# sdoira/U96-SLAM

Measured on AMD Instinct MI355X. Metric: Mpix-disparities/s, higher is better.
Workload: dtype u8

## Files before the change

### u96-slam_amd/csrc/sbm_api.hip

```cpp
#include <stdio.h>
#include <stdlib.h>
#include <string.h>

#include <algorithm>
#include <mutex>
#include <new>

#include "sbm_handle.h"

using namespace sbm;

enum BmStage { kBmPrefilter, kBmSad, kBmBorder, kBmLr, kBmSpeckle, kBmTotal, kBmStageCount };
enum BmMark { kBmBegin, kBmPrefiltered, kBmMatched, kBmChecked, kBmEnd, kBmMarkCount };
static const char* const kBmNames[] = {"prefilter", "sad", "border", "lrcheck", "speckle", "total"};
StageTable sbm::bm_stages() { return stage_table<kBmStageCount, 0>(kBmNames); }
static_assert(kBmMarkCount == sbm_handle::kMarks, "the ring holds one event per mark");

extern "C" {

void sbm_params_default(sbm_params* p, int num_disparities, int block_size) {
  if (!p) return;
  memset(p, 0, sizeof(*p));
  p->prefilter_type = SBM_PREFILTER_XSOBEL;
  p->prefilter_size = 9;
// ... 275 lines not shown
    pl->sad = wide ? kSadWide : kSadGeneric;
    snprintf(pl->kernel, sizeof(pl->kernel), "%s",
             !wide ? "sad_generic_kernel" : (pl->in_envelope ? "sad_wide_kernel [in-place accumulate unavailable]" : "sad_wide_kernel"));
  }
  pl->speckle = p.speckle_range >= 0 && p.speckle_window_size > 0;
  if (pl->speckle) {
    speckle_plan(g, p.speckle_window_size, p.speckle_range, &pl->spk);
    size_t part[4];
    SpeckleScratch::bytes(g.n, g.W, g.H, part);
    for (int i = 0; i < 4; i++) pl->spk_bytes[i] = (long long)part[i];
  }
}

extern "C" {

static int ensure_scratch(sbm_handle* h, int n, int W, int H, int pitch, bool need_cost, bool need_speckle) {
  auto& s = h->bm;
  const bool fits = n <= s.n && W == s.W && H == s.H && pitch == s.pitch && s.pf_l.p;
  if (!fits) {
    HIPCHK(h, hipStreamSynchronize(h->stream));
    release_set(s);
    const size_t npix = (size_t)n * W * H, pfbytes = (size_t)n * pitch * H + 4096;
    HIPCHK(h, s.pf_l.grow(pfbytes, h->stream));
    HIPCHK(h, s.pf_r.grow(pfbytes, h->stream));
    HIPCHK(h, s.disp_pre.grow(npix * sizeof(int16_t), h->stream));
    HIPCHK(h, hipMemsetAsync(s.pf_l.p, 0, pfbytes, h->stream));
    HIPCHK(h, hipMemsetAsync(s.pf_r.p, 0, pfbytes, h->stream));
    s.n = n; s.W = W; s.H = H; s.pitch = pitch;
  }
  const size_t npix = (size_t)s.n * W * H;
  if (need_cost) HIPCHK(h, s.cost.grow(npix * sizeof(int32_t), h->stream));
  HIPCHK(h, s.lr_keys.grow(lr_keys_bytes(s.n, W, H, need_cost), h->stream));
  if (need_speckle) HIPCHK(h, s.spk.ensure(s.n, W, H, h->stream));
  return SBM_OK;
}

static inline void mark(sbm_handle* h, BmMark i) {
  if (h->instr) hipEventRecord(h->ev[h->calls % sbm_handle::kRing][i], h->stream);
}

static void collect_profile(sbm_handle* h) {
  unsigned nrec = std::min<unsigned>(h->calls, sbm_handle::kRing), first = 0;
  if (h->profiling == 1 && h->calls > 0) { first = (h->calls - 1) % sbm_handle::kRing; nrec = 1; }
  static const BmStage kStage[kBmMarkCount - 1] = {kBmPrefilter, kBmSad, kBmLr, kBmSpeckle};
  float acc[kBmMarkCount - 1] = {}, tot = 0.f;
  for (unsigned r = first; r < first + nrec; r++) {
    for (int i = 0; i < kBmMarkCount - 1; i++) {
      float ms = 0.f;
// ... 9 lines not shown

int sbm_compute_device(sbm_handle* h, int n, const void* d_left, const void* d_right, int width, int height,
                       void* d_disp, int sync) {
  if (!h || !d_left || !d_right || !d_disp) return SBM_ERR_NULL;
  if (n <= 0) return SBM_ERR_BATCH;
  const sbm_params& p = h->p;
  BmPlan pl;
  const int st = bm_plan_geom(p, n, width, height, &pl);
  if (st != SBM_OK) return st;
  DeviceScope dscope(h->device);
  HIPCHK(h, dscope.enter());
  bool inplace = false;
  if (pl.in_envelope) HIPCHK(h, mqsad_inplace_ok(h->stream, &inplace));
  bm_plan_launches(p, inplace, &pl);
  const Geom& g = pl.g;
  const int st2 = ensure_scratch(h, n, width, height, g.pitch, g.want_cost, pl.speckle);
  if (st2 != SBM_OK) return st2;
  h->last = g; h->have_last = true;
  if (pl.any_rows) snprintf(h->last_kernel, sizeof(h->last_kernel), "%s", pl.kernel);

  const uint8_t* dl = (const uint8_t*)d_left;
  const uint8_t* dr = (const uint8_t*)d_right;
  uint8_t *pf_l = h->bm.pf_l.as<uint8_t>(), *pf_r = h->bm.pf_r.as<uint8_t>();
  int16_t* disp_pre = h->bm.disp_pre.as<int16_t>();
  int32_t* cost = h->bm.cost.as<int32_t>();
  int16_t* out = (int16_t*)d_disp;

  h->instr = h->profiling && h->ev_ok && (h->profiling != 3 || (h->ncall & 3u) == 0);
  mark(h, kBmBegin);
  if (pl.any_rows) {
    if (p.prefilter_type == SBM_PREFILTER_XSOBEL) {
      HIPCHK(h, launch_prefilter(dl, dr, pf_l, pf_r, g, h->stream));
    } else {
      HIPCHK(h, h->bm.vsum.grow((size_t)2 * h->bm.n * width * height * sizeof(uint16_t), h->stream));
      HIPCHK(h, launch_prefilter_norm(dl, dr, pf_l, pf_r, h->bm.vsum.as<uint16_t>(), g, p.prefilter_size, h->stream));
    }
  }
  mark(h, kBmPrefiltered);
  if (pl.sad == kSadFast) {
    HIPCHK(h, launch_sad_fast(pf_l, pf_r, disp_pre, cost, pl, h->stream));
    if (pl.wide_borders) {
      HIPCHK(h, launch_sad_wide(pf_l, pf_r, disp_pre, cost, g, pl.wide_l[0], pl.wide_l[1], h->stream));
      HIPCHK(h, launch_sad_wide(pf_l, pf_r, disp_pre, cost, g, pl.wide_r[0], pl.wide_r[1], h->stream));
    }
  } else if (pl.sad == kSadWide) {
    HIPCHK(h, launch_sad_wide(pf_l, pf_r, disp_pre, cost, g, 0, g.xend, h->stream));
  } else if (pl.sad == kSadGeneric) {
    HIPCHK(h, launch_sad_generic(pf_l, pf_r, disp_pre, cost, g, 0, g.xend, h->stream));
  }
  mark(h, kBmMatched);
  HIPCHK(h, launch_lrcheck(disp_pre, cost, out, h->bm.lr_keys.as<unsigned long long>(), g, p.disp12_max_diff, h->stream));
  mark(h, kBmChecked);
  if (pl.speckle) HIPCHK(h, launch_speckle(out, h->bm.spk, g, pl.spk, p.speckle_window_size, h->stream));
  mark(h, kBmEnd);
  if (h->instr) h->calls++;
// ... 153 lines not shown
    return SBM_OK;
  }
  if (which == 3) {
    if (dst_bytes < npix * sizeof(int16_t)) return SBM_ERR_SIZE;
    HIPCHK(h, hipMemcpy(dst, h->bm.disp_pre.p, npix * sizeof(int16_t), hipMemcpyDeviceToHost));
    int16_t* d = (int16_t*)dst;
    for (int i = 0; i < g.n; i++)
      for (int y = 0; y < g.H; y++) {
        int16_t* row = d + ((size_t)i * g.H + y) * g.W;
        const bool live = y >= g.row0 && y < g.row1;
        for (int x = 0; x < g.W; x++)
          if (!live || x < g.lofs || x >= g.lofs + g.xend) row[x] = (int16_t)g.filtered;
      }
    return SBM_OK;
  }
  return SBM_ERR_UNSUPPORTED;
}

}
```

### u96-slam_amd/csrc/sbm_common.h

```cpp
#pragma once
#include <hip/hip_runtime.h>
#include <stdint.h>

#include "../../include/sbm.h"

#include <stdlib.h>

namespace sbm {

inline int env_switch(const char* name, int dflt) {
  const char* e = getenv(name);
  return e ? atoi(e) : dflt;
}

struct Geom {
  int W, H;
  int n;
  int pitch;
  int padl;
  int plane;
  int nd, mindisp, wsz, w2, cap;
  int lofs, rofs, width1, xend;
  int tex, uniq;
  int filtered;
// ... 61 lines not shown
};
int bm_plan_geom(const sbm_params& p, int n, int W, int H, BmPlan* pl);
void bm_plan_launches(const sbm_params& p, bool inplace_ok, BmPlan* pl);
inline int bm_plan(const sbm_params& p, int n, int W, int H, bool inplace_ok, BmPlan* pl) {
  const int st = bm_plan_geom(p, n, W, H, pl);
  if (st == SBM_OK) bm_plan_launches(p, inplace_ok, pl);
  return st;
}

bool sad_fast_supported(const Geom& g);
hipError_t mqsad_inplace_ok(hipStream_t s, bool* ok);
constexpr int kFastNdMax = 512;
bool sad_fast_borders_in_launch(const Geom& g);
int sad_fast_pfshift(const Geom& g);
void sad_fast_plan(BmPlan* pl);
hipError_t launch_sad_fast(const uint8_t* pf_l, const uint8_t* pf_r, int16_t* disp, int32_t* cost, BmPlan& pl, hipStream_t s);

constexpr int kLrLdsCols = 8192;
inline size_t lr_keys_bytes(int n, int W, int H, bool do_lr) {
  return do_lr && W > kLrLdsCols ? (size_t)n * H * W * sizeof(unsigned long long) : 0;
}
hipError_t launch_lrcheck(const int16_t* disp_pre, const int32_t* cost, int16_t* disp_out, unsigned long long* keys,
                          const Geom& g, int disp12_max_diff, hipStream_t s);

constexpr int kSpkMaxSeg = 4, kSpkRecordPad = 288, kSpkSeamPad = 512;
void speckle_plan(const Geom& g, int max_size, int max_diff, SpkPlan* k);

hipError_t launch_prefilter_dense(const uint8_t* d_src, uint8_t* d_dst, int n, int W, int H, int rtl, int cap,
                                  hipStream_t s);
hipError_t launch_rect_map(const sbm_rect_cam& cam, int W, int H, int16_t* d_map, hipStream_t s);
hipError_t launch_rect_remap(const uint8_t* d_src, const int16_t* d_map, uint8_t* d_dst, int n, int W, int H,
// ... 23 lines not shown
```

### u96-slam_amd/csrc/sbm_handle.h

```cpp
#pragma once
#include <string.h>

#include "sbm_common.h"

#define HIPCHK(h, call)                         \
  do {                                          \
    hipError_t e_ = (call);                     \
    if (e_ != hipSuccess) {                     \
      (h)->last_hip = (int)e_;                  \
      return e_ == hipErrorOutOfMemory ? SBM_ERR_NOMEM : SBM_ERR_HIP; \
    }                                           \
  } while (0)

struct DeviceScope {
  int prev, dev;
  bool have;
  explicit DeviceScope(int d) : prev(-1), dev(d), have(false) { have = hipGetDevice(&prev) == hipSuccess; }
  hipError_t enter() { return (have && prev == dev) ? hipSuccess : hipSetDevice(dev); }
  ~DeviceScope() {
    if (have && prev != dev) hipSetDevice(prev);
  }
};

namespace sbm {
// ... 88 lines not shown

}

struct sbm_handle {
  sbm_params p;
  int device;
  hipStream_t stream;
  int last_hip;
  struct {
    int n, W, H, pitch;
    sbm::DevBuf pf_l, pf_r;
    sbm::DevBuf disp_pre;
    sbm::DevBuf cost;
    sbm::DevBuf lr_keys;
    sbm::DevBuf vsum;
    sbm::SpeckleScratch spk;
    sbm::StageClock clock;
    template <class F> void each(F f) { f(pf_l); f(pf_r); f(disp_pre); f(cost); f(lr_keys); f(vsum); spk.each(f); }
  } bm;
  struct {
    int n, W, H;
    int gen;
    sbm::DevBuf rec, flag, xs_l, xs_r;
    template <class F> void each(F f) { f(rec); f(flag); f(xs_l); f(xs_r); }
  } fp;
  struct {
    int n, W, H;
    sbm::DevBuf l, r, d;
    sbm::DevBuf zc_cnt;
    template <class F> void each(F f) { f(l); f(r); f(d); f(zc_cnt); }
  } st;
  uint8_t* pin;
  size_t pin_bytes;
// ... 106 lines not shown
```

### u96-slam_amd/csrc/sbm_sad_fast.hip

```cpp
#include <string.h>

#include "sbm_sad_fast_kernel.h"

namespace sbm {

__global__ void __launch_bounds__(256) mqsad_inplace_selftest_kernel(unsigned* bad) {
  unsigned long long st = (unsigned long long)(blockIdx.x * 256 + threadIdx.x) * 0x9E3779B97F4A7C15ull + 88172645463325252ull;
  auto rnd = [&]() { st ^= st << 13; st ^= st >> 7; st ^= st << 17; return st; };
  unsigned nbad = 0;
  for (int it = 0; it < 64; it++) {
    unsigned long long accA[4], accR[4], win[4];
    const unsigned pat = (unsigned)rnd() & ((it & 1) ? 0x00ffffffu : 0x000000ffu);
#pragma unroll
    for (int q = 0; q < 4; q++) { accA[q] = accR[q] = rnd() & 0x3fff3fff3fff3fffull; win[q] = rnd(); }
#pragma unroll
    for (int r = 0; r < 3; r++)
#pragma unroll
      for (int q = 0; q < 4; q++) {
        accR[q] = __builtin_amdgcn_mqsad_pk_u16_u8(win[(q + r) & 3], pat, accR[q]);
        asm volatile("v_mqsad_pk_u16_u8 %0, %1, %2, %0" : "+v"(accA[q]) : "v"(win[(q + r) & 3]), "v"(pat));
      }
#pragma unroll
    for (int q = 0; q < 4; q++) nbad += accA[q] != accR[q];
  }
// ... 59 lines not shown
  if (g.row0 < g.w2 || g.row1 > g.H - g.w2 || g.row1 <= g.row0) return false;
  if ((long)g.plane * 4 >= (1L << 31)) return false;
  const int xhi = std::min(g.W - g.lofs - 1, g.W - g.rofs - g.nd);
  if (xhi - g.w2 + 1 <= g.w2) return false;
  return true;
}

static hipError_t sad_fast_dispatch(BmPlan& pl, const FastArgs* a, hipStream_t s) {
  switch (pl.g.wsz) {
    case 15: return launch_nd<5, 3>(pl, a, s);
    case 21: return launch_nd<7, 3>(pl, a, s);
    default: return launch_sad_fast_pw1(pl, a, s);
  }
}

void sad_fast_plan(BmPlan* pl) {
  const Geom& g = pl->g;
  FastPlan& a = pl->f;
  const int xhi = std::min(g.W - g.lofs - 1, g.W - g.rofs - g.nd);
  a.xc0 = g.w2; a.xc1 = xhi - g.w2 + 1;
  const int pw = g.wsz % 3 == 0 ? 3 : 1;
  const int nv = 64 - (g.wsz - pw);
  const int cs3_env = env_switch("SBM_FAST_CS3", 1);
  const int ncols = a.xc1 - a.xc0;
  const int nv3 = 64 - (g.wsz / 3 - 1);
  int triples = 0;
  if (pw == 3 && cs3_env) {
    triples = ncols / (3 * nv3);
    if (ncols - triples * 3 * nv3 > 2 * nv) triples++;
  }
  a.strips3 = 3 * triples;
  const int rem = std::max(0, ncols - triples * 3 * nv3);
  const int strips = a.strips3 + (rem + nv - 1) / nv;
  const int rows = g.row1 - g.row0;
  const int round1 = g.nd <= 256 ? 1536 : (g.nd <= 384 ? 1024 : 768);
  constexpr double kSegC = 0.196;
  int nseg = 1;
  {
    const double prime = 0.2 * (g.wsz - 1);
    const double slots = g.nd <= 64 ? 4096.0 : (g.nd <= 128 ? 3072.0 : (double)round1);
    nseg = (int)(std::sqrt(kSegC * slots * rows / ((double)strips * g.n * prime)) + 0.5);
    nseg = std::max(1, std::min(nseg, std::max(1, rows / g.wsz)));
  }
  constexpr int kSmallRows = 8;
  constexpr long kFill = 5000;
  const int maxseg = std::max(nseg, std::min(64, rows / kSmallRows));
  const long per_seg = (long)strips * g.n;
  if (per_seg * maxseg * (g.nd > 128 ? (g.nd + 127) / 128 : 1) < 1800) {
    nseg = std::max(nseg, (int)std::min<long>(maxseg, 1023 / per_seg));
  } else {
    const int nseg1 = nseg;
    while (per_seg * nseg < kFill && nseg < maxseg) nseg++;
    if (g.nd > 128 && per_seg * nseg > round1 && 2 * per_seg * nseg < 3 * round1) nseg = std::max(nseg1, (int)((long)round1 * 1450 / 1536 / per_seg));
  }
  nseg = std::min(nseg, 64);
  int ns = 0;
  a.segrow[0] = g.row0;
  if (nseg < 3) {
    const int seg = (rows + nseg - 1) / nseg;
    for (int y = g.row0; y < g.row1; y += seg) a.segrow[++ns] = std::min(y + seg, g.row1);
  } else {
    const double unit = rows / (nseg - 1.5);
    double acc = 0;
    for (int k = 0; k < nseg; k++) {
      const double wgt = k < nseg - 3 ? 1.0 : (k == nseg - 3 ? 0.75 : (k == nseg - 2 ? 0.5 : 0.25));
      acc += wgt * unit;
      const int y = k == nseg - 1 ? g.row1 : std::min(g.row1, g.row0 + (int)(acc + 0.5));
      if (y > a.segrow[ns]) a.segrow[++ns] = y;
    }
  }
  nseg = ns;
  a.strips = strips; a.nseg = nseg;
  {
    const long maxs = (long)g.wsz * g.wsz * 2 * g.cap;
    a.uniq_plain = 8 * ((maxs * g.uniq / 100 + 1) << g.pfshift) <= 65535;
  }
  a.split = (long)strips * nseg * g.n < 1024;
  sad_fast_dispatch(*pl, nullptr, nullptr);
}

hipError_t launch_sad_fast(const uint8_t* pf_l, const uint8_t* pf_r, int16_t* disp, int32_t* cost, BmPlan& pl, hipStream_t s) {
  const Geom& g = pl.g;
  const FastPlan& f = pl.f;
  FastArgs a;
  a.pf_l = pf_l; a.pf_r = pf_r; a.disp = disp; a.cost = g.want_cost ? reinterpret_cast<uint16_t*>(cost) : nullptr;
  a.W = g.W; a.H = g.H; a.pitch = g.pitch; a.padl = g.padl; a.plane = g.plane;
  a.nd = g.nd; a.mindisp = g.mindisp; a.lofs = g.lofs; a.rofs = g.rofs; a.tex = g.tex << g.pfshift; a.uniq = g.uniq;
  a.filtered = g.filtered; a.capb = (g.cap << g.pfshift) + kPfBias; a.pfshift = g.pfshift;
  a.row0 = g.row0; a.row1 = g.row1;
  static_assert(sizeof(a.segrow) == sizeof(f.segrow), "");
  memcpy(a.segrow, f.segrow, sizeof(a.segrow));
  a.strips = f.strips; a.nseg = f.nseg; a.npairs = g.n; a.strips3 = f.strips3; a.uniq_plain = f.uniq_plain;
  a.xc0 = f.xc0; a.xc1 = f.xc1;
  a.bord = f.bord; a.bnw = f.bnw; a.bseg = f.bseg; a.nbseg = f.nbseg;
  return sad_fast_dispatch(pl, &a, s);
}

}
```

### u96-slam_amd/csrc/sbm_sad_fast_core.h

```cpp
#pragma once
#include <stdio.h>
#include <stdlib.h>

#include <algorithm>
#include <cmath>
#include <mutex>
#include <type_traits>

#include "sbm_common.h"

namespace sbm {

typedef unsigned int u32;
typedef unsigned long long u64;
typedef unsigned short u16x2 __attribute__((ext_vector_type(2)));
typedef unsigned int u32x4 __attribute__((ext_vector_type(4)));

struct FastArgs {
  const uint8_t* pf_l;
  const uint8_t* pf_r;
  int16_t* disp;
  uint16_t* cost;
  int W, H, pitch, padl, plane;
  int nd, mindisp, lofs, rofs, tex, uniq, filtered, capb;
  int row0, row1;
  int segrow[66];
  int strips, nseg, npairs;
  int strips3;
  int uniq_plain;
  int xc0, xc1;
  int pfshift;
  int bord;
  int bnw;
  int bseg, nbseg;
};

__device__ __forceinline__ u32 pk_sub_sat(u32 a, u32 b) {
  u16x2 r = __builtin_elementwise_sub_sat(__builtin_bit_cast(u16x2, a), __builtin_bit_cast(u16x2, b));
  return __builtin_bit_cast(u32, r);
}
__device__ __forceinline__ u32 pk_add_sat(u32 a, u32 b) {
  u16x2 r = __builtin_elementwise_add_sat(__builtin_bit_cast(u16x2, a), __builtin_bit_cast(u16x2, b));
  return __builtin_bit_cast(u32, r);
}
__device__ __forceinline__ u32 pk_min(u32 a, u32 b) {
  u16x2 r = __builtin_elementwise_min(__builtin_bit_cast(u16x2, a), __builtin_bit_cast(u16x2, b));
  return __builtin_bit_cast(u32, r);
}
__device__ __forceinline__ u32 umin3(u32 a, u32 b, u32 c) {
  u32 r;
  asm("v_min3_u32 %0, %1, %2, %3" : "=v"(r) : "v"(a), "v"(b), "v"(c));
  return r;
}

extern __shared__ __attribute__((aligned(16))) uint4 fast_lds[];

#include "sbm_sad_border_wave.h"

constexpr int kFastPrioExchange = 2;

template <int NDW, int NTERM, int PW, int CS>
struct FastLds {
  static constexpr int NQ = NDW / 4;
  static constexpr int NCH = (NQ + 15) / 16;
  static constexpr int NSLOT = ((CS * 63 + 4 + 16 * (4 * (NCH - 1) + 3) + 1) + 63) / 64 * 64;
  static constexpr int KS = CS == 3 ? 1 : PW;
  static constexpr int XS = 64 + KS * (NTERM - 1);
  static_assert(CS == 1 || (CS == 3 && PW == 3), "column stride 3 goes with 3-column sums");
// ... 162 lines not shown
```

### u96-slam_amd/csrc/sbm_sad_fast_kernel.h

```cpp
#pragma once
#include "sbm_sad_fast_core.h"
#include "sbm_sad_fast_strip.h"

namespace sbm {

template <int NDW, int NWAVES, int NTERM, int PW, bool EXACT_ND, bool DUAL>
__global__ void __launch_bounds__(64 * NWAVES) __attribute__((amdgpu_waves_per_eu(NDW > 64 ? 3 : (NWAVES > 2 ? 5 : 4))))
sad_fast_kernel(FastArgs a) {
  const int bpp = a.strips;
  int strip, segi, pair;
  {
    if constexpr (NDW * NWAVES <= 256) {
    if ((int)blockIdx.x < a.bord * a.nbseg) {
      using BL = BorderLds<(PW * NTERM) / 2, NDW * NWAVES>;
      const int bseg = blockIdx.x / a.bord, b = blockIdx.x - bseg * a.bord;
      const int wv = NWAVES > 1 ? __builtin_amdgcn_readfirstlane(threadIdx.x >> 6) : 0;
      const int wi = b * NWAVES + wv;
      if (wi < a.bnw) sad_border_wave<(PW * NTERM) / 2, NDW * NWAVES>(a, reinterpret_cast<unsigned char*>(fast_lds) + wv * BL::BYTES, bseg, wi);
      return;
    }
    }
    const int sid = blockIdx.x - a.bord * a.nbseg;
    const int per_seg = a.strips * a.npairs;
    segi = sid / per_seg;
    const int b = sid - segi * per_seg;
    const int full = (a.npairs / 8) * 8 * bpp;
    int p, inner;
    if (b < full) {
      const int xcd = b & 7, k = b >> 3;
      p = (k / bpp) * 8 + xcd;
      inner = k % bpp;
    } else {
      const int r = b - full;
      p = (a.npairs / 8) * 8 + r / bpp;
      inner = r % bpp;
    }
    pair = p;
    strip = inner;
  }
  const int wvk = NWAVES > 1 ? __builtin_amdgcn_readfirstlane(threadIdx.x >> 6) : 0;
  unsigned char* const ldsb = reinterpret_cast<unsigned char*>(fast_lds);
  auto strip_at = [&](auto cs_tag, const int cb) {
    constexpr int CSV = decltype(cs_tag)::value;
    using D = DmaLds<NDW, NWAVES, NTERM, PW, CSV>;
    unsigned char* const wb = ldsb + wvk * D::WAVE_B;
    unsigned char* const xl = wb + 2 * D::AREA_B;
    sad_fast_strip_dma<NDW, NWAVES, NTERM, PW, EXACT_ND, CSV>(a, wb, wb + D::AREA_B, xl,
                                                            reinterpret_cast<u32*>(ldsb + NWAVES * D::WAVE_B), cb, segi, pair);
  };
  if constexpr (DUAL) {
    constexpr int NV3 = 64 - (NTERM - 1), NV1 = 64 - PW * (NTERM - 1);
    if (strip < a.strips3) {
      const int t = strip / 3;
      strip_at(std::integral_constant<int, 3>{}, t * (3 * NV3) + (strip - 3 * t));
    } else {
      strip_at(std::integral_constant<int, 1>{}, (a.strips3 / 3) * (3 * NV3) + (strip - a.strips3) * NV1);
    }
  } else {
    constexpr int NV1 = 64 - PW * (NTERM - 1);
    strip_at(std::integral_constant<int, 1>{}, strip * NV1);
  }
}

// ... 22 lines not shown
      int bseg = (int)(kBorderChainShare * t_kernel_us / t_row_us - 0.25 * (wsz - 1));
      bseg = std::max(4, std::min(bseg, rows));
      f.nbseg = (rows + bseg - 1) / bseg;
      f.bseg = (rows + f.nbseg - 1) / f.nbseg;
      f.nbseg = (rows + f.bseg - 1) / f.bseg;
    }
    f.grid = f.bord * f.nbseg + f.strips * g.n * f.nseg;
    f.block = 64 * NWAVES;
    f.lds = (int)lds;
    f.NDW = NDW; f.NWAVES = NWAVES; f.NTERM = NTERM; f.PW = PW; f.dual = DUAL;
    f.exact = HAS_EXACT && g.nd == NDW * NWAVES;
    snprintf(pl.kernel, sizeof(pl.kernel), "sad_fast_kernel<%d,%d,%d,%d,%s,%s> pfshift=%d",
             NDW, NWAVES, NTERM, PW, f.exact ? "true" : "false", DUAL ? "true" : "false", g.pfshift);
    return hipSuccess;
  }
  const dim3 grid((unsigned)pl.f.grid);
  const size_t lds = (size_t)pl.f.lds;
  if constexpr (HAS_EXACT) {
    if (pl.f.exact) {
      hipLaunchKernelGGL((sad_fast_kernel<NDW, NWAVES, NTERM, PW, true, DUAL>), grid, dim3(64 * NWAVES), lds, s, *a);
      return hipGetLastError();
    }
  }
    hipLaunchKernelGGL((sad_fast_kernel<NDW, NWAVES, NTERM, PW, false, DUAL>), grid, dim3(64 * NWAVES), lds, s, *a);
  return hipGetLastError();
}

template <int NTERM, int PW>
static hipError_t launch_nd(BmPlan& pl, const FastArgs* a, hipStream_t s) {
  const int nd = pl.g.nd;
  const bool split = pl.f.split;
// ... 17 lines not shown
```

### u96-slam_amd/csrc/sbm_sad_fast_strip.h

```cpp
#pragma once
#include "sbm_sad_fast_core.h"

namespace sbm {

template <int NDW, int NWAVES, int NTERM, int PW, bool EXACT_ND, int CS>
__device__ __forceinline__ void sad_fast_strip_dma(const FastArgs& a, unsigned char* __restrict__ const b0c, unsigned char* __restrict__ const b1c,
                                                   unsigned char* __restrict__ const xl1c,
                                                   u32* __restrict__ const xkey,
                                                   const int cbase, const int segi, const int pair) {
  using L = FastLds<NDW, NTERM, PW, CS>;
  using D = DmaLds<NDW, NWAVES, NTERM, PW, CS>;
  using P = HPlan<NTERM, PW>;
  typedef __attribute__((address_space(3))) void* lds_vptr;
  constexpr int NQ = NDW / 4;
  constexpr int NR = NDW / 2;
  constexpr int NSLOT = L::NSLOT;
  constexpr int NIT = NSLOT / 64;
  constexpr int WSZ = PW * NTERM, W2 = WSZ / 2;
  constexpr int KS = L::KS;
  constexpr int NV = 64 - KS * (NTERM - 1);
  constexpr int XCH = D::XCH, XS = L::XS;

  const int lane = threadIdx.x & 63;
  const int wv = NWAVES > 1 ? __builtin_amdgcn_readfirstlane(threadIdx.x >> 6) : 0;
  const int d0 = wv * NDW;
  const int ndl = EXACT_ND ? NDW : a.nd - d0;
  const int c = cbase + CS * lane;
  const int xc = c + W2;
  const bool produces = lane < NV && xc >= a.xc0 && xc < a.xc1;
  const int ys = a.segrow[segi];
  const int ye = a.segrow[segi + 1];
  const uint8_t* pl = a.pf_l + (size_t)pair * a.plane + a.padl + a.lofs + cbase;
  const uint8_t* pr = a.pf_r + (size_t)pair * a.plane + a.padl + a.rofs + cbase + d0;
  uint2* const xacc = reinterpret_cast<uint2*>(xkey + 2 * NWAVES * 64);
  const unsigned lane_u = (unsigned)lane;
  const __amdgpu_buffer_rsrc_t rs_l = __builtin_amdgcn_make_buffer_rsrc(const_cast<uint8_t*>(pl), 0, 0x7fffffff, 0x00020000);
  const __amdgpu_buffer_rsrc_t rs_r = __builtin_amdgcn_make_buffer_rsrc(const_cast<uint8_t*>(pr), 0, 0x7fffffff, 0x00020000);
  uint4* const b0 = reinterpret_cast<uint4*>(b0c);
  uint4* const b1 = reinterpret_cast<uint4*>(b1c);
  uint4* const xq0 = b0;
  uint4* const xq1 = reinterpret_cast<uint4*>(xl1c);
  auto xt_of = [](uint4* const xq) { return reinterpret_cast<u32*>(xq + (XCH / 2) * XS); };
  const u32 capw = (u32)a.capb * 0x01010101u;

  u64 VB[NQ];
  {
    const u32 unit = (lane_u / (unsigned)KS) % (unsigned)NTERM == 0u ? FastTag<WSZ>::tag_unit(a.pfshift) : 0u;
#pragma unroll
    for (int q = 0; q < NQ; q++) {
      const u32 tq = (u32)((2 * q) / (NR / FastTag<WSZ>::NGRP)) * unit;
      VB[q] = __builtin_bit_cast(u64, make_uint2(tq, tq));
    }
  }
  u32 Vt = 0;

  auto pat_of = [](uint4* const buf) { return reinterpret_cast<u32*>(reinterpret_cast<unsigned char*>(buf) + D::PAT_OFS); };
// ... 49 lines not shown
  #pragma unroll
        for (int g = 0; g < NQ / 4; g++) {
          if (16 * g < ndl) {
            u32 lo[4], hi[4];
  #pragma unroll
            for (int k = 0; k < 4; k++) { lo[k] = win4[4 * (4 * g + k)]; hi[k] = win4[4 * (4 * g + k) + 4]; }
  #pragma unroll
            for (int k = 0; k < 4; k++) quad(4 * g + k, lo[k], hi[k]);
          }
        }
      }
    }
    Vt = leave ? Vt - tv : Vt + tv;
  };

  stage(ys - W2, b0);
  for (int i = 0; i < 2 * W2; i += 2) {
    landed();
    stage(ys - W2 + i + 1, b1);
    apply(b0, false);
    landed();
    stage(ys - W2 + i + 2, b0);
    apply(b1, false);
  }
  const __amdgpu_buffer_rsrc_t rs_d = __builtin_amdgcn_make_buffer_rsrc(a.disp + (size_t)pair * a.W * a.H, 0, 0x7fffffff, 0x00020000);
  const __amdgpu_buffer_rsrc_t rs_c = __builtin_amdgcn_make_buffer_rsrc(a.cost + (size_t)pair * a.W * a.H, 0, 0x7fffffff, 0x00020000);
  const int ocol_u = __builtin_amdgcn_readfirstlane(2 * (a.lofs + cbase + W2));
  u32 res_prev = 0xffff0000u;
  auto flush = [&](const int yrow) {
    if (produces && (NWAVES == 1 || (yrow % NWAVES) == wv)) {
      const int orow_prev = __builtin_amdgcn_readfirstlane(2 * yrow * a.W) + ocol_u;
      u32 l3 = CS * lane_u;
      asm volatile("" : "+v"(l3));
      const int ocol = (int)(2 * l3);
      if (a.cost) __builtin_amdgcn_raw_buffer_store_b16((short)(res_prev >> 16), rs_c, ocol, orow_prev, 0);
      __builtin_amdgcn_raw_buffer_store_b16((short)res_prev, rs_d, ocol, orow_prev, 0);
    }
  };
// ... 29 lines not shown
        A[e][0] = v0.x; A[e][1] = v0.y; A[e][2] = v1.x; A[e][3] = v1.y;
        xq0[e * XS + lane] = make_uint4(v0.x, v0.y, v1.x, v1.y);
      }
      if (tex_now) xt_of(xq0)[lane] = Vt;
      published();
      if constexpr (P::S1 > 1) {
#pragma unroll
        for (int e = 0; e < XCH / 2; e++)
#pragma unroll
          for (int k = 1; k < P::S1; k++) add4(A[e], xq0[e * XS + lx + KS * k]);
        if (tex_now)
#pragma unroll
          for (int k = 1; k < P::S1; k++) tA += xt_of(xq0)[lx + KS * k];
        if constexpr (P::PUB1) {
#pragma unroll
          for (int e = 0; e < XCH / 2; e++) xq1[e * XS + lane] = make_uint4(A[e][0], A[e][1], A[e][2], A[e][3]);
          if (tex_now) xt_of(xq1)[lane] = tA;
          published();
        }
      }
      {
        constexpr int OV = P::NTT * P::S1;
#pragma unroll
        for (int e = 0; e < XCH / 2; e++) {
#pragma unroll
          for (int t = 1; t < P::NTT; t++) add4(A[e], xq1[e * XS + lx + KS * P::S1 * t]);
#pragma unroll
          for (int v = (P::NTT > 0 ? 0 : 1); v < P::NVV; v++) add4(A[e], xq0[e * XS + lx + KS * (OV + v)]);
        }
        if (tex_now) {
#pragma unroll
          for (int t = 1; t < P::NTT; t++) tA += xt_of(xq1)[lx + KS * P::S1 * t];
#pragma unroll
          for (int v = (P::NTT > 0 ? 0 : 1); v < P::NVV; v++) tA += xt_of(xq0)[lx + KS * (OV + v)];
          tex_ok = __ballot((int)tA >= a.tex);
        }
      }
#pragma unroll
      for (int e = 0; e < XCH / 2; e++)
#pragma unroll
        for (int i = 0; i < 4; i++) S[2 * (q0 + 2 * e) + i] = A[e][i];
// ... 50 lines not shown
      }
    }

    bool ok = __builtin_amdgcn_inverse_ballot_w64(tex_ok);
    if (a.uniq > 0) ok = ok && fast_unique(acc_lo, acc_hi, T, minsad, mind, nn, pp, a.nd);
    if (mine && produces) {
      int out = a.filtered, cst = -1;
      if (ok) {
        out = fast_subpixel(nn, pp, minsad, mind, a.nd, a.mindisp);
        if (a.cost) cst = minsad >> a.pfshift;
      }
      res_prev = ((u32)out & 0xffffu) | ((u32)cst << 16);
    }
  }
  flush(ye - 1);
}

}
```

### u96-slam_amd/stereobm.py

```python
import ctypes

import numpy as np

from . import _engine, _fpga, _frontend, _gftt, _lk, _match, _orb, _pnp
from ._abi import (PNP_FEW_MATCHES, PNP_FEW_RANSAC_INLIERS, PNP_FEW_REFINED_INLIERS, PNP_HYP_DTYPE, PNP_NO_MODEL, PNP_OK,
                   PNP_RESULT_DTYPE, PREFILTER_FLAVOUR_CV, PREFILTER_FLAVOUR_RTL, PREFILTER_NORMALIZED_RESPONSE, PREFILTER_XSOBEL,
                   FpgaParams, GfttCvParams, GfttSelectParams, LK_GET_MIN_EIGENVALS, LK_USE_INITIAL_FLOW, LkParams, MatchParams, OrbParams, PnpParams, RectCam, SbmParams, StereoBMError,
                   StereoModel, _check, library_path, load_library, loaded_library_name)
from ._fpga import fpga_params, fpga_params_from_regs, fpga_sad_size_reg, fpga_validate
from ._frontend import make_rect_cam
from ._gftt import gftt_cv_params, gftt_cv_validate, gftt_select_capacity, gftt_select_params, gftt_select_validate
from ._lk import lk_level_sizes, lk_params, lk_validate
from ._match import match_params, match_validate
from ._orb import orb_params, orb_pattern_array, orb_validate
from ._pnp import pnp_params, pnp_records, pnp_validate


class StereoBM(_engine.Engine, _frontend.FrontEnd, _fpga.FpgaMatcher, _gftt.Gftt, _orb.Orb, _match.Match, _pnp.Pnp, _lk.Lk):

    def __init__(self, numDisparities=0, blockSize=21, device=0):
        L = load_library()
        self._p = SbmParams()
        L.sbm_params_default(ctypes.byref(self._p), numDisparities, blockSize)
        self._open(L, self._p, device)
# ... 105 lines not shown

    def launch_raw(self, n, d_left, d_right, w, h, d_disp, sync=False):
        _check(self._L.sbm_compute_device(self._h, n, d_left, d_right, w, h, d_disp, 1 if sync else 0), self._h)

    def stream(self):
        return self._L.sbm_stream(self._h)

    def last_kernel(self):
        buf = ctypes.create_string_buffer(128)
        _check(self._L.sbm_last_kernel_name(self._h, buf, 128), self._h)
        return buf.value.decode()

    def profile(self):
        return self._profile(("prefilter", "sad", "lrcheck", "speckle", "total"))

    def debug_fetch(self, which, n, h, w):
        dt = {0: np.uint8, 1: np.uint8, 2: np.int32, 3: np.int16}[which]
        a = np.empty((n, h, w), dt)
        _check(self._L.sbm_debug_fetch(self._h, which, a.ctypes.data, a.nbytes), self._h)
        return a


def compute_multi(engines, left, right, disparity):
    for a, dt in ((left, np.uint8), (right, np.uint8), (disparity, np.int16)):
        if not isinstance(a, np.ndarray) or a.dtype != dt or a.ndim != 3 or not a.flags.c_contiguous:
            raise StereoBMError(-2, "compute_multi takes C-contiguous (n,H,W) arrays: uint8 images, int16 disparity")
    if left.shape != right.shape or left.shape != disparity.shape:
        raise StereoBMError(-2, "All the images must have the same size")
    if not engines:
        raise StereoBMError(-24, "compute_multi needs at least one engine")
    n, h, w = left.shape
    L = load_library()
    hs = (ctypes.c_void_p * len(engines))(*[e._h for e in engines])
# ... 11 lines not shown
```

Baseline: 4.300 million.

## Hand off SAD column-sum state between row segments to skip priming

Each row-segment block of the fast SAD kernel normally re-primes its vertical window sums by streaming 2*W2 rows. Now a block that finishes a segment stores its running column sums to a global handoff buffer and publishes an epoch flag. The block for the next segment loads that state if the flag is already set, and falls back to priming otherwise. Segments are reordered and their lengths reweighted so that later-scheduled segments can find their predecessor finished. This adds global traffic, flag memsets and atomics, and relies on block scheduling order for the shortcut to apply.

Result: faster. 4.357 million (median of 6 runs) (+1.3%).

```diff
diff --git a/u96-slam_amd/csrc/sbm_api.hip b/u96-slam_amd/csrc/sbm_api.hip
--- a/u96-slam_amd/csrc/sbm_api.hip
+++ b/u96-slam_amd/csrc/sbm_api.hip
@@ -313,7 +313,8 @@
 
 extern "C" {
 
-static int ensure_scratch(sbm_handle* h, int n, int W, int H, int pitch, bool need_cost, bool need_speckle) {
+static int ensure_scratch(sbm_handle* h, int n, int W, int H, int pitch, bool need_cost, bool need_speckle, size_t ho_bytes,
+                          size_t ho_flags) {
   auto& s = h->bm;
   const bool fits = n <= s.n && W == s.W && H == s.H && pitch == s.pitch && s.pf_l.p;
   if (!fits) {
@@ -331,6 +332,15 @@
   if (need_cost) HIPCHK(h, s.cost.grow(npix * sizeof(int32_t), h->stream));
   HIPCHK(h, s.lr_keys.grow(lr_keys_bytes(s.n, W, H, need_cost), h->stream));
   if (need_speckle) HIPCHK(h, s.spk.ensure(s.n, W, H, h->stream));
+  if (ho_bytes) {
+    const bool fresh = ho_bytes > s.handoff.bytes;
+    HIPCHK(h, s.handoff.grow(ho_bytes, h->stream));
+    if (fresh || ho_flags != s.ho_flags || s.ho_epoch == 0xffffffffu) {
+      HIPCHK(h, hipMemsetAsync(s.handoff.p, 0, ho_flags, h->stream));
+      s.ho_flags = ho_flags;
+      s.ho_epoch = 0;
+    }
+  }
   return SBM_OK;
 }
 
@@ -370,9 +380,12 @@
   if (pl.in_envelope) HIPCHK(h, mqsad_inplace_ok(h->stream, &inplace));
   bm_plan_launches(p, inplace, &pl);
   const Geom& g = pl.g;
-  const int st2 = ensure_scratch(h, n, width, height, g.pitch, g.want_cost, pl.speckle);
+  size_t ho_flags = 0;
+  const size_t ho_bytes = sad_fast_handoff_bytes(pl, &ho_flags);
+  const int st2 = ensure_scratch(h, n, width, height, g.pitch, g.want_cost, pl.speckle, ho_bytes, ho_flags);
   if (st2 != SBM_OK) return st2;
   h->last = g; h->have_last = true;
+  h->bm.ho_links = 0;
   if (pl.any_rows) snprintf(h->last_kernel, sizeof(h->last_kernel), "%s", pl.kernel);
 
   const uint8_t* dl = (const uint8_t*)d_left;
@@ -394,7 +407,9 @@
   }
   mark(h, kBmPrefiltered);
   if (pl.sad == kSadFast) {
-    HIPCHK(h, launch_sad_fast(pf_l, pf_r, disp_pre, cost, pl, h->stream));
+    h->bm.ho_slots = (size_t)(pl.f.nseg - 1) * g.n * pl.f.strips;
+    HIPCHK(h, launch_sad_fast(pf_l, pf_r, disp_pre, cost, pl, ho_bytes ? h->bm.handoff.p : nullptr, ho_bytes ? ++h->bm.ho_epoch : 0u,
+                              &h->bm.ho_links, h->stream));
     if (pl.wide_borders) {
       HIPCHK(h, launch_sad_wide(pf_l, pf_r, disp_pre, cost, g, pl.wide_l[0], pl.wide_l[1], h->stream));
       HIPCHK(h, launch_sad_wide(pf_l, pf_r, disp_pre, cost, g, pl.wide_r[0], pl.wide_r[1], h->stream));
@@ -578,6 +593,22 @@
       }
     return SBM_OK;
   }
+  if (which == 7) {
+    if (dst_bytes < 2 * sizeof(int32_t)) return SBM_ERR_SIZE;
+    int32_t* d = (int32_t*)dst;
+    d[0] = 0;
+    d[1] = (int32_t)h->bm.ho_links;
+    if (!h->bm.ho_links) return SBM_OK;
+    const size_t slots = h->bm.ho_slots;
+    uint32_t* tmp = (uint32_t*)malloc(slots * sizeof(uint32_t));
+    if (!tmp) return SBM_ERR_NOMEM;
+    const hipError_t e = hipMemcpy(tmp, h->bm.handoff.as<uint32_t>() + slots, slots * sizeof(uint32_t), hipMemcpyDeviceToHost);
+    if (e == hipSuccess)
+      for (size_t i = 0; i < slots; i++) d[0] += tmp[i] == h->bm.ho_epoch;
+    free(tmp);
+    HIPCHK(h, e);
+    return SBM_OK;
+  }
   return SBM_ERR_UNSUPPORTED;
 }
 
diff --git a/u96-slam_amd/csrc/sbm_common.h b/u96-slam_amd/csrc/sbm_common.h
--- a/u96-slam_amd/csrc/sbm_common.h
+++ b/u96-slam_amd/csrc/sbm_common.h
@@ -99,7 +99,9 @@
 bool sad_fast_borders_in_launch(const Geom& g);
 int sad_fast_pfshift(const Geom& g);
 void sad_fast_plan(BmPlan* pl);
-hipError_t launch_sad_fast(const uint8_t* pf_l, const uint8_t* pf_r, int16_t* disp, int32_t* cost, BmPlan& pl, hipStream_t s);
+size_t sad_fast_handoff_bytes(const BmPlan& pl, size_t* flag_bytes);
+hipError_t launch_sad_fast(const uint8_t* pf_l, const uint8_t* pf_r, int16_t* disp, int32_t* cost, BmPlan& pl, void* handoff,
+                           unsigned epoch, long* links, hipStream_t s);
 
 constexpr int kLrLdsCols = 8192;
 inline size_t lr_keys_bytes(int n, int W, int H, bool do_lr) {
diff --git a/u96-slam_amd/csrc/sbm_handle.h b/u96-slam_amd/csrc/sbm_handle.h
--- a/u96-slam_amd/csrc/sbm_handle.h
+++ b/u96-slam_amd/csrc/sbm_handle.h
@@ -126,9 +126,14 @@
     sbm::DevBuf cost;
     sbm::DevBuf lr_keys;
     sbm::DevBuf vsum;
+    sbm::DevBuf handoff;
+    size_t ho_flags;
+    unsigned ho_epoch;
+    size_t ho_slots;
+    long ho_links;
     sbm::SpeckleScratch spk;
     sbm::StageClock clock;
-    template <class F> void each(F f) { f(pf_l); f(pf_r); f(disp_pre); f(cost); f(lr_keys); f(vsum); spk.each(f); }
+    template <class F> void each(F f) { f(pf_l); f(pf_r); f(disp_pre); f(cost); f(lr_keys); f(vsum); f(handoff); spk.each(f); }
   } bm;
   struct {
     int n, W, H;
diff --git a/u96-slam_amd/csrc/sbm_sad_fast.hip b/u96-slam_amd/csrc/sbm_sad_fast.hip
--- a/u96-slam_amd/csrc/sbm_sad_fast.hip
+++ b/u96-slam_amd/csrc/sbm_sad_fast.hip
@@ -97,6 +97,23 @@
   }
 }
 
+static int fast_handoff_mode() { return std::max(0, std::min(2, env_switch("SBM_FAST_HANDOFF", 1))); }
+
+static int fast_slots(int nd) { return nd <= 64 ? 4096 : 3072; }
+
+constexpr double kFirstRoundStep = 0.10, kFirstRoundSpan = 0.40;
+
+static int fast_segment_order(int nseg, long per_seg, int slots, int nd, unsigned char* at) {
+  for (int k = 0; k < 64; k++) at[k] = (unsigned char)k;
+  if (fast_handoff_mode() != 1 || nd > 128) return nseg;
+  const long D = (slots + per_seg - 1) / per_seg + 1;
+  if (D >= nseg) return nseg;
+  int base = 0;
+  for (int r = 0; r < (int)D; r++)
+    for (int p = r; p < nseg; p += (int)D) at[p] = (unsigned char)base++;
+  return (int)D;
+}
+
 void sad_fast_plan(BmPlan* pl) {
   const Geom& g = pl->g;
   FastPlan& a = pl->f;
@@ -118,10 +135,11 @@
   const int rows = g.row1 - g.row0;
   const int round1 = g.nd <= 256 ? 1536 : (g.nd <= 384 ? 1024 : 768);
   constexpr double kSegC = 0.196;
+  const int slots_i = g.nd <= 64 ? 4096 : (g.nd <= 128 ? 3072 : round1);
   int nseg = 1;
   {
     const double prime = 0.2 * (g.wsz - 1);
-    const double slots = g.nd <= 64 ? 4096.0 : (g.nd <= 128 ? 3072.0 : (double)round1);
+    const double slots = slots_i;
     nseg = (int)(std::sqrt(kSegC * slots * rows / ((double)strips * g.n * prime)) + 0.5);
     nseg = std::max(1, std::min(nseg, std::max(1, rows / g.wsz)));
   }
@@ -143,14 +161,36 @@
     const int seg = (rows + nseg - 1) / nseg;
     for (int y = g.row0; y < g.row1; y += seg) a.segrow[++ns] = std::min(y + seg, g.row1);
   } else {
-    const double unit = rows / (nseg - 1.5);
-    double acc = 0;
-    for (int k = 0; k < nseg; k++) {
-      const double wgt = k < nseg - 3 ? 1.0 : (k == nseg - 3 ? 0.75 : (k == nseg - 2 ? 0.5 : 0.25));
-      acc += wgt * unit;
-      const int y = k == nseg - 1 ? g.row1 : std::min(g.row1, g.row0 + (int)(acc + 0.5));
-      if (y > a.segrow[ns]) a.segrow[++ns] = y;
+    unsigned char at[64];
+    const int stride = fast_segment_order(nseg, per_seg, slots_i, g.nd, at);
+    const int first_round = stride - 1;
+    int len[64];
+    {
+      const double step = first_round > 1 ? std::min(kFirstRoundStep, kFirstRoundSpan / (first_round - 1)) : 0.0;
+      double wgt[64], sum = 0;
+      for (int p = 0; p < nseg; p++) {
+        wgt[p] = p < nseg - 3 ? 1.0 : (p == nseg - 3 ? 0.75 : (p == nseg - 2 ? 0.5 : 0.25));
+        if (stride < nseg && p < first_round) wgt[p] = std::min(wgt[p], 1.0 - step * (first_round - 1 - p));
+        sum += wgt[p];
+      }
+      const double unit = rows / sum;
+      double acc = 0;
+      int y0 = 0;
+      for (int p = 0; p < nseg; p++) {
+        acc += wgt[p] * unit;
+        const int y1 = p == nseg - 1 ? rows : std::min(rows, (int)(acc + 0.5));
+        len[p] = y1 - y0;
+        y0 = y1;
+      }
     }
+    int np = 0;
+    for (int p = 0; p < nseg; p++)
+      if (len[p] > 0) len[np++] = len[p];
+    fast_segment_order(np, per_seg, slots_i, g.nd, at);
+    int seglen[64];
+    for (int p = 0; p < np; p++) seglen[at[p]] = len[p];
+    for (int k = 0; k < np; k++) a.segrow[k + 1] = a.segrow[k] + seglen[k];
+    ns = np;
   }
   nseg = ns;
   a.strips = strips; a.nseg = nseg;
@@ -162,7 +202,31 @@
   sad_fast_dispatch(*pl, nullptr, nullptr);
 }
 
-hipError_t launch_sad_fast(const uint8_t* pf_l, const uint8_t* pf_r, int16_t* disp, int32_t* cost, BmPlan& pl, hipStream_t s) {
+static unsigned long long fast_handoff_links(const BmPlan& pl, unsigned char* at) {
+  const FastPlan& f = pl.f;
+  const int mode = fast_handoff_mode();
+  const int stride = fast_segment_order(f.nseg, (long)f.strips * pl.g.n, fast_slots(pl.g.nd), pl.g.nd, at);
+  if (mode == 0 || f.NWAVES != 1 || !f.exact || f.nseg < 2) return 0;
+  unsigned long long links = 0;
+  for (int p = mode == 2 ? 1 : stride; p < f.nseg; p++) links |= 1ull << at[p];
+  return links;
+}
+
+constexpr size_t kHandoffMaxBytes = (size_t)1 << 30;
+size_t sad_fast_handoff_bytes(const BmPlan& pl, size_t* flag_bytes) {
+  unsigned char at[64];
+  *flag_bytes = 0;
+  if (!pl.fast || !fast_handoff_links(pl, at)) return 0;
+  const size_t slots = (size_t)(pl.f.nseg - 1) * pl.g.n * pl.f.strips;
+  const size_t fb = (2 * slots * sizeof(u32) + 255) & ~(size_t)255;
+  const size_t bytes = fb + slots * ((size_t)(pl.f.NDW / 4) * 512 + 256);
+  if (bytes > kHandoffMaxBytes) return 0;
+  *flag_bytes = fb;
+  return bytes;
+}
+
+hipError_t launch_sad_fast(const uint8_t* pf_l, const uint8_t* pf_r, int16_t* disp, int32_t* cost, BmPlan& pl, void* handoff,
+                           unsigned epoch, long* links, hipStream_t s) {
   const Geom& g = pl.g;
   const FastPlan& f = pl.f;
   FastArgs a;
@@ -176,7 +240,21 @@
   a.strips = f.strips; a.nseg = f.nseg; a.npairs = g.n; a.strips3 = f.strips3; a.uniq_plain = f.uniq_plain;
   a.xc0 = f.xc0; a.xc1 = f.xc1;
   a.bord = f.bord; a.bnw = f.bnw; a.bseg = f.bseg; a.nbseg = f.nbseg;
-  return sad_fast_dispatch(pl, &a, s);
-}
-
-}
+  a.ho_link = fast_handoff_links(pl, a.segat);
+  if (!handoff) a.ho_link = 0;
+  a.ho = static_cast<u32*>(handoff); a.ho_epoch = epoch;
+  a.segbase = 0; a.grid = f.grid;
+  const long per_seg = (long)f.strips * g.n;
+  *links = (long)__builtin_popcountll(a.ho_link) * per_seg;
+  if (fast_handoff_mode() != 2 || !a.ho_link) return sad_fast_dispatch(pl, &a, s);
+  for (int k = 0; k < f.nseg; k++) {
+    a.segbase = k;
+    a.grid = (int)per_seg + (k == 0 ? f.bord * f.nbseg : 0);
+    if (k == 1) a.bord = 0;
+    const hipError_t e = sad_fast_dispatch(pl, &a, s);
+    if (e != hipSuccess) return e;
+  }
+  return hipSuccess;
+}
+
+}
diff --git a/u96-slam_amd/csrc/sbm_sad_fast_core.h b/u96-slam_amd/csrc/sbm_sad_fast_core.h
--- a/u96-slam_amd/csrc/sbm_sad_fast_core.h
+++ b/u96-slam_amd/csrc/sbm_sad_fast_core.h
@@ -15,6 +15,7 @@
 typedef unsigned long long u64;
 typedef unsigned short u16x2 __attribute__((ext_vector_type(2)));
 typedef unsigned int u32x4 __attribute__((ext_vector_type(4)));
+typedef unsigned int u32x2 __attribute__((ext_vector_type(2)));
 
 struct FastArgs {
   const uint8_t* pf_l;
@@ -26,6 +27,12 @@
   int row0, row1;
   int segrow[66];
   int strips, nseg, npairs;
+  unsigned char segat[64];
+  int grid;
+  int segbase;
+  unsigned long long ho_link;
+  u32* ho;
+  u32 ho_epoch;
   int strips3;
   int uniq_plain;
   int xc0, xc1;
@@ -52,6 +59,13 @@
   asm("v_min3_u32 %0, %1, %2, %3" : "=v"(r) : "v"(a), "v"(b), "v"(c));
   return r;
 }
+
+constexpr int kHandoffAux = 16;
+template <int NDW, int NWAVES, bool EXACT_ND>
+struct FastHandoff {
+  static constexpr bool ON = NWAVES == 1 && EXACT_ND;
+  static constexpr int SLOT_B = (NDW / 4) * 512 + 256;
+};
 
 extern __shared__ __attribute__((aligned(16))) uint4 fast_lds[];
 
diff --git a/u96-slam_amd/csrc/sbm_sad_fast_kernel.h b/u96-slam_amd/csrc/sbm_sad_fast_kernel.h
--- a/u96-slam_amd/csrc/sbm_sad_fast_kernel.h
+++ b/u96-slam_amd/csrc/sbm_sad_fast_kernel.h
@@ -22,8 +22,9 @@
     }
     const int sid = blockIdx.x - a.bord * a.nbseg;
     const int per_seg = a.strips * a.npairs;
-    segi = sid / per_seg;
-    const int b = sid - segi * per_seg;
+    const int pos = sid / per_seg;
+    segi = a.segat[a.segbase + pos];
+    const int b = sid - pos * per_seg;
     const int full = (a.npairs / 8) * 8 * bpp;
     int p, inner;
     if (b < full) {
@@ -46,7 +47,7 @@
     unsigned char* const wb = ldsb + wvk * D::WAVE_B;
     unsigned char* const xl = wb + 2 * D::AREA_B;
     sad_fast_strip_dma<NDW, NWAVES, NTERM, PW, EXACT_ND, CSV>(a, wb, wb + D::AREA_B, xl,
-                                                            reinterpret_cast<u32*>(ldsb + NWAVES * D::WAVE_B), cb, segi, pair);
+                                                            reinterpret_cast<u32*>(ldsb + NWAVES * D::WAVE_B), cb, segi, pair, strip);
   };
   if constexpr (DUAL) {
     constexpr int NV3 = 64 - (NTERM - 1), NV1 = 64 - PW * (NTERM - 1);
@@ -99,7 +100,7 @@
              NDW, NWAVES, NTERM, PW, f.exact ? "true" : "false", DUAL ? "true" : "false", g.pfshift);
     return hipSuccess;
   }
-  const dim3 grid((unsigned)pl.f.grid);
+  const dim3 grid((unsigned)a->grid);
   const size_t lds = (size_t)pl.f.lds;
   if constexpr (HAS_EXACT) {
     if (pl.f.exact) {
diff --git a/u96-slam_amd/csrc/sbm_sad_fast_strip.h b/u96-slam_amd/csrc/sbm_sad_fast_strip.h
--- a/u96-slam_amd/csrc/sbm_sad_fast_strip.h
+++ b/u96-slam_amd/csrc/sbm_sad_fast_strip.h
@@ -7,7 +7,7 @@
 __device__ __forceinline__ void sad_fast_strip_dma(const FastArgs& a, unsigned char* __restrict__ const b0c, unsigned char* __restrict__ const b1c,
                                                    unsigned char* __restrict__ const xl1c,
                                                    u32* __restrict__ const xkey,
-                                                   const int cbase, const int segi, const int pair) {
+                                                   const int cbase, const int segi, const int pair, const int strip) {
   using L = FastLds<NDW, NTERM, PW, CS>;
   using D = DmaLds<NDW, NWAVES, NTERM, PW, CS>;
   using P = HPlan<NTERM, PW>;
@@ -20,6 +20,7 @@
   constexpr int KS = L::KS;
   constexpr int NV = 64 - KS * (NTERM - 1);
   constexpr int XCH = D::XCH, XS = L::XS;
+  constexpr bool HANDOFF = FastHandoff<NDW, NWAVES, EXACT_ND>::ON;
 
   const int lane = threadIdx.x & 63;
   const int wv = NWAVES > 1 ? __builtin_amdgcn_readfirstlane(threadIdx.x >> 6) : 0;
@@ -40,6 +41,7 @@
   uint4* const b1 = reinterpret_cast<uint4*>(b1c);
   uint4* const xq0 = b0;
   uint4* const xq1 = reinterpret_cast<uint4*>(xl1c);
+  typedef u32x4 __attribute__((may_alias)) u32x4a;
   auto xt_of = [](uint4* const xq) { return reinterpret_cast<u32*>(xq + (XCH / 2) * XS); };
   const u32 capw = (u32)a.capb * 0x01010101u;
 
@@ -119,14 +121,38 @@
     Vt = leave ? Vt - tv : Vt + tv;
   };
 
-  stage(ys - W2, b0);
-  for (int i = 0; i < 2 * W2; i += 2) {
-    landed();
-    stage(ys - W2 + i + 1, b1);
-    apply(b0, false);
-    landed();
-    stage(ys - W2 + i + 2, b0);
-    apply(b1, false);
+  const size_t ho_slots = HANDOFF ? (size_t)(a.nseg - 1) * a.npairs * a.strips : 0;
+  const size_t ho_mine = HANDOFF ? ((size_t)segi * a.npairs + pair) * a.strips + strip : 0;
+  auto ho_rsrc = [&](const size_t slot) {
+    unsigned char* const p = reinterpret_cast<unsigned char*>(a.ho) + ((2 * ho_slots * sizeof(u32) + 255) & ~(size_t)255) + slot * FastHandoff<NDW, NWAVES, EXACT_ND>::SLOT_B;
+    return __builtin_amdgcn_make_buffer_rsrc(p, 0, FastHandoff<NDW, NWAVES, EXACT_ND>::SLOT_B, 0x00020000);
+  };
+  bool take = false;
+  if constexpr (HANDOFF) {
+    if ((a.ho_link >> segi) & 1) {
+      const size_t from = ho_mine - (size_t)a.npairs * a.strips;
+      take = __builtin_amdgcn_readfirstlane(__hip_atomic_load(a.ho + from, __ATOMIC_RELAXED, __HIP_MEMORY_SCOPE_AGENT)) == a.ho_epoch;
+      if (take) {
+        __builtin_amdgcn_fence(__ATOMIC_ACQUIRE, "agent");
+        const __amdgpu_buffer_rsrc_t rs_h = ho_rsrc(from);
+#pragma unroll
+        for (int q = 0; q < NQ; q++) VB[q] = __builtin_bit_cast(u64, __builtin_amdgcn_raw_buffer_load_b64(rs_h, (int)(8 * lane_u), 512 * q, kHandoffAux));
+        Vt = __builtin_amdgcn_raw_buffer_load_b32(rs_h, (int)(4 * lane_u), 512 * NQ, kHandoffAux);
+        if (lane == 0) a.ho[ho_slots + from] = a.ho_epoch;
+        stage(ys + W2, b0);
+      }
+    }
+  }
+  if (!take) {
+    stage(ys - W2, b0);
+    for (int i = 0; i < 2 * W2; i += 2) {
+      landed();
+      stage(ys - W2 + i + 1, b1);
+      apply(b0, false);
+      landed();
+      stage(ys - W2 + i + 2, b0);
+      apply(b1, false);
+    }
   }
   const __amdgpu_buffer_rsrc_t rs_d = __builtin_amdgcn_make_buffer_rsrc(a.disp + (size_t)pair * a.W * a.H, 0, 0x7fffffff, 0x00020000);
   const __amdgpu_buffer_rsrc_t rs_c = __builtin_amdgcn_make_buffer_rsrc(a.cost + (size_t)pair * a.W * a.H, 0, 0x7fffffff, 0x00020000);
@@ -186,7 +212,10 @@
           for (int k = 1; k < P::S1; k++) tA += xt_of(xq0)[lx + KS * k];
         if constexpr (P::PUB1) {
 #pragma unroll
-          for (int e = 0; e < XCH / 2; e++) xq1[e * XS + lane] = make_uint4(A[e][0], A[e][1], A[e][2], A[e][3]);
+          for (int e = 0; e < XCH / 2; e++) {
+            if constexpr (HANDOFF) *reinterpret_cast<u32x4a*>(xq1 + e * XS + lane) = (u32x4){A[e][0], A[e][1], A[e][2], A[e][3]};
+            else xq1[e * XS + lane] = make_uint4(A[e][0], A[e][1], A[e][2], A[e][3]);
+          }
           if (tex_now) xt_of(xq1)[lane] = tA;
           published();
         }
@@ -196,7 +225,14 @@
 #pragma unroll
         for (int e = 0; e < XCH / 2; e++) {
 #pragma unroll
-          for (int t = 1; t < P::NTT; t++) add4(A[e], xq1[e * XS + lx + KS * P::S1 * t]);
+          for (int t = 1; t < P::NTT; t++) {
+            if constexpr (HANDOFF) {
+              const u32x4 r = *reinterpret_cast<const u32x4a*>(xq1 + e * XS + lx + KS * P::S1 * t);
+              add4(A[e], make_uint4(r.x, r.y, r.z, r.w));
+            } else {
+              add4(A[e], xq1[e * XS + lx + KS * P::S1 * t]);
+            }
+          }
 #pragma unroll
           for (int v = (P::NTT > 0 ? 0 : 1); v < P::NVV; v++) add4(A[e], xq0[e * XS + lx + KS * (OV + v)]);
         }
@@ -277,6 +313,18 @@
     }
   }
   flush(ye - 1);
+  if constexpr (HANDOFF) {
+    if (segi + 1 < a.nseg && ((a.ho_link >> (segi + 1)) & 1)) {
+      landed();
+      apply(b1, true);
+      const __amdgpu_buffer_rsrc_t rs_h = ho_rsrc(ho_mine);
+#pragma unroll
+      for (int q = 0; q < NQ; q++) __builtin_amdgcn_raw_buffer_store_b64(__builtin_bit_cast(u32x2, VB[q]), rs_h, (int)(8 * lane_u), 512 * q, kHandoffAux);
+      __builtin_amdgcn_raw_buffer_store_b32(Vt, rs_h, (int)(4 * lane_u), 512 * NQ, kHandoffAux);
+      asm volatile("s_waitcnt vmcnt(0)" ::: "memory");
+      if (lane == 0) __hip_atomic_store(a.ho + ho_mine, a.ho_epoch, __ATOMIC_RELAXED, __HIP_MEMORY_SCOPE_AGENT);
+    }
+  }
 }
 
 }
diff --git a/u96-slam_amd/stereobm.py b/u96-slam_amd/stereobm.py
--- a/u96-slam_amd/stereobm.py
+++ b/u96-slam_amd/stereobm.py
@@ -143,9 +143,9 @@
     def profile(self):
         return self._profile(("prefilter", "sad", "lrcheck", "speckle", "total"))
 
-    def debug_fetch(self, which, n, h, w):
-        dt = {0: np.uint8, 1: np.uint8, 2: np.int32, 3: np.int16}[which]
-        a = np.empty((n, h, w), dt)
+    def debug_fetch(self, which, n=0, h=0, w=0):
+        dt = {0: np.uint8, 1: np.uint8, 2: np.int32, 3: np.int16, 7: np.int32}[which]
+        a = np.empty((2,) if which == 7 else (n, h, w), dt)
         _check(self._L.sbm_debug_fetch(self._h, which, a.ctypes.data, a.nbytes), self._h)
         return a
 
```
